# noway/nzcp-circom

Measured on AMD Instinct MI355X. Metric: groth16_proofs_per_sec_nzcp_live, higher is better.
Workload: dtype u32x8 (256-bit Montgomery integers); 1 GPU; nzcp_liveTest.circom = NZCPPubIdentity(1, 355, 0, 4, 2, 4, 6), single proof: nVars=825434, nConstraints=830227, nPublic=513, domain=2^20, nCoefs=4236306; parallelism=1gpu

## Files before the change

nzcp-circom_amd/csrc/internal.h:

```cpp
#pragma once
#include <hip/hip_runtime.h>
#include <stddef.h>
#include <stdint.h>
#include <stdlib.h>
#include <string.h>
#include <functional>
#include <memory>
#include <new>
#include <string>
#include <vector>

#include "../../include/g16_prover.h"
#include "device_job.h"
#include "ec.cuh"
#include "fq29.cuh"

struct g16_prover;
namespace g16 {

void set_error(const std::string& msg);
const char* get_error();

#define G16_HIP(expr)                                                                      \
  do {                                                                                     \
// ... 196 lines not shown
  uint64_t max_entries = 0;
};
size_t msm_point_bytes(int curve);
int msm_group_create(MsmGroup& g, const MsmSectionIn* secs, int nsec, const MsmConfig& cfg);
struct MsmWorkspaceDelete { void operator()(MsmWorkspace* ws) const; };
using MsmWorkspacePtr = std::unique_ptr<MsmWorkspace, MsmWorkspaceDelete>;
int msm_workspace_create(MsmWorkspacePtr& ws, const MsmGroup& g);
static constexpr int kMsmPrioHighest = -1000;
void msm_set_aux_stream_priority(int prio);
struct MsmResult {
  G1XYZZ g1[kMsmMaxSections];
  G2XYZZ g2;
};
static constexpr uint32_t kDupMin = 8;
static constexpr uint32_t kDupChunkBits = 16;
int msm_launch(const MsmGroup& g, MsmWorkspace* ws, const Fr* d_scalars, hipStream_t st, hipStream_t st2);
int msm_launch_front(const MsmGroup& g, MsmWorkspace* ws, const Fr* d_scalars, hipStream_t st);
int msm_launch_lanes(const MsmGroup& g, MsmWorkspace* ws, hipStream_t st, hipStream_t st2, hipEvent_t gate1,
                     hipEvent_t gate2);
void msm_set_quota(MsmWorkspace* ws, uint32_t quota_g1, uint32_t quota_g2);
hipEvent_t msm_event(MsmWorkspace* ws, int which);
int msm_collect(const MsmGroup& g, MsmWorkspace* ws, MsmResult* out,
                const std::function<void(const MsmResult&)>* after_g1 = nullptr);
double trace_ms();
float msm_last_accum_ms(const MsmWorkspace* ws, int lane);
void msm_set_throughput(MsmWorkspace* ws, const MsmGroup& g, bool on);
void msm_set_waves(MsmWorkspace* ws, uint32_t waves_g1, uint32_t waves_g2);
float msm_event_offset_ms(MsmWorkspace* ws, hipEvent_t base, int lane, int which);

template <class F> inline void msm_combine_windows(XYZZ<F>& total, const XYZZ<F>* windows, int W, int c, bool ones) {
  xyzz_set_inf(total);
  for (int j = W - 1; j >= 0; j--) {
    if (!xyzz_is_inf(total))
      for (int k = 0; k < c; k++) xyzz_dbl(total);
    xyzz_add(total, windows[j]);
  }
  if (ones) xyzz_add(total, windows[W]);
}
template <class F> inline void msm_add_bit_sums(XYZZ<F>& total, const XYZZ<F>* bits, uint32_t chunk_bits, uint32_t nrows) {
  XYZZ<F> acc;
  xyzz_set_inf(acc);
  for (int b = (int)nrows - 1; b >= 0; b--) {
    if (!xyzz_is_inf(acc))
      for (uint32_t k = 0; k < chunk_bits; k++) xyzz_dbl(acc);
    xyzz_add(acc, bits[b]);
  }
  xyzz_add(total, acc);
}
// ... 3 lines not shown
```

nzcp-circom_amd/csrc/msm.cuh:

```cuda
#pragma once
#include <stdlib.h>

#include <atomic>

#include "ec29.cuh"
#include "internal.h"

namespace g16 {

struct MsmPlan {
  uint32_t nsec, n;
  uint32_t sec_begin[kMsmMaxSections];
  int c, Ws;
  uint32_t W, pf, B, low_bits, bins, rps, rows, ones;
  uint32_t salt_bits;
  uint32_t dup_rows, dup_bits;
  uint32_t wb, wx;
  uint32_t wkb;
};
__host__ __device__ __forceinline__ uint32_t msm_win_off(const MsmPlan& pl, uint32_t j) { return j * pl.wb + (j < pl.wx ? j : pl.wx); }
__host__ __device__ __forceinline__ uint32_t msm_win_bits(const MsmPlan& pl, uint32_t j) { return pl.wb + (j < pl.wx ? 1u : 0u); }

__host__ __device__ __forceinline__ uint32_t msm_dup_hash(const uint32_t x[8], uint32_t bits) {
  uint64_t h = 0x9E3779B97F4A7C15ull;
// ... 29 lines not shown
  DeviceBuf<uint4> d_qdesc;
  DeviceBuf<uint32_t> d_class;
  DeviceBuf<uint32_t> d_queue;
  DeviceBuf<uint32_t> d_redo;
  DeviceBuf<void> d_partial;
  DeviceBuf<void> d_bsum;
  DeviceBuf<uint32_t> d_heavy;
  DeviceBuf<uint32_t> d_medium;
  uint32_t max_heavy = 0;
  DeviceBuf<void> d_seg;
  DeviceBuf<void> d_red;
  bool reduce_scan = false;
  void* d_canon = nullptr;
  DeviceBuf<void> d_canon_own;
  DeviceBuf<void> d_dseg;
  DeviceBuf<void> d_dred;
  DeviceEvent ev_dup_fork, ev_dup_join;
  DeviceBuf<uint32_t> d_dcount;
  DeviceBuf<uint32_t> d_dlist;
  uint32_t nsec_lane = 0;
  PinnedBuf<uint8_t> h_pinned;
  bool rows_mapped = false;
  size_t out_bytes = 0;
  DeviceEvent ev0, ev1;
  DeviceEvent ev_done;
  DeviceEvent trace_ev[4];
  DeviceStream st_dup;
  float last_accum_ms = 0.f;
  hipEvent_t gate = nullptr;
  uint32_t waves_per_simd = 0;
  uint32_t chunk_quota = 0;
};

struct MsmWorkspace {
  DeviceBuf<uint32_t> d_hist;
  DeviceBuf<uint32_t> d_bin_cnt;
  DeviceBuf<uint32_t> d_bin_start;
  DeviceBuf<uint2> d_tmp;
  DeviceBuf<uint32_t> d_sorted;
  DeviceBuf<uint32_t> d_cnt;
  uint32_t nb = 0;
  DeviceBuf<uint32_t> d_dup_cnt;
  DeviceBuf<uint32_t> d_dup_rep;
  DeviceBuf<uint32_t> d_dup_mixed;
  const Fr* d_scalars = nullptr;
  bool direct = false;
  uint32_t bin_cap = 0;
  uint32_t dup_chunk = 16, dup_bit_rows = 16;
  PinnedBuf<uint32_t> h_over;
  hipStream_t st_last = nullptr, st2_last = nullptr;
  MsmLaneWs lane[2];
// ... 728 lines not shown
  static_assert(sizeof(TPT) == sizeof(PT), "tail ops must share the point layout");
  static const bool trace = getenv("G16_TRACE_HOST") != nullptr;
  auto mark = [&](int k) {
    if (!trace) return;
    if (!ln.trace_ev[k]) (void)ln.trace_ev[k].create();
    (void)hipEventRecord(ln.trace_ev[k], st);
  };
  int rc = msm_build_queue(g, ws, ln, st);
  if (rc) return rc;
  mark(0);
  const uint32_t nbk = ln.key_hi - ln.key_lo;
  const uint32_t full_occ = (uint32_t)F::kAccumWavesPerSimd;
  const uint32_t occ = (ln.waves_per_simd && ln.waves_per_simd < full_occ) ? ln.waves_per_simd : full_occ;
  uint64_t waves = (uint64_t)256 * 4 * occ;
  const uint64_t max_chunks = (ln.max_tasks + kTaskChunk - 1) / kTaskChunk;
  uint32_t quota = 0xffffffffu;
  if (ln.chunk_quota) {
    quota = ln.chunk_quota;
    waves = (max_chunks + quota - 1) / quota + 64;
  }
  if (waves > max_chunks) waves = max_chunks;
  if (waves == 0) waves = 1;
  if (ln.gate) G16_HIP(hipStreamWaitEvent(st, ln.gate, 0));
  G16_HIP(hipEventRecord(ln.ev0, st));
  msm_accumulate_kernel<F><<<(unsigned)waves, 64, 0, st>>>((const PackedAffine<F>*)d_bases, ws->d_sorted, ln.d_toff, nbk,
                                                            ln.point_base, ln.d_qdesc, ln.d_queue, ln.d_redo,
                                                            (PT*)ln.d_partial, quota);
  G16_HIP(hipEventRecord(ln.ev1, st));
  msm_redo_kernel<F><<<64, 64, 0, st>>>((const PackedAffine<F>*)d_bases, ws->d_sorted, ln.point_base, ln.d_task_desc,
                                        ln.d_queue, ln.d_redo, (PT*)ln.d_partial);
  msm_combine_light_kernel<FT><<<(nbk + kTailThreads - 1) / kTailThreads, kTailThreads, 0, st>>>((const TPT*)ln.d_partial, ln.d_toff, nbk,
                                                              (TPT*)ln.d_bsum, ln.d_heavy, ln.max_heavy, ln.d_medium,
                                                              msm_light_max(ln), ln.h_stat);
  msm_combine_medium_kernel<FT><<<1024, kTailThreads, 0, st>>>((const TPT*)ln.d_partial, ln.d_toff, (TPT*)ln.d_bsum, ln.d_medium,
                                                              ln.max_heavy);
  msm_combine_heavy_kernel<FT><<<2048, kTailThreads, 0, st>>>((const TPT*)ln.d_partial, ln.d_toff, (TPT*)ln.d_bsum,
                                                   ln.d_heavy, ln.max_heavy);
  mark(1);
  uint32_t nout_pts = ln.row_pts;
  if (g.dup_rows) {
    hipStream_t sd = ln.st_dup ? ln.st_dup : st;
    if (sd != st) {
      G16_HIP(hipEventRecord(ln.ev_dup_fork, st));
      G16_HIP(hipStreamWaitEvent(sd, ln.ev_dup_fork, 0));
    }
    const uint32_t nchunk = (1u << g.dup_bits) >> 6, drows = ln.nsec_lane * ws->dup_bit_rows;
    const uint32_t waves_d = drows * nchunk;
    const uint32_t sec0 = ln.key_lo / (g.rps * g.B), dup_row0 = (uint32_t)g.W + (g.ones ? 1u : 0u);
    G16_HIP(hipMemsetAsync(ln.d_dcount, 0, 16, sd));
    msm_dup_compact_kernel<<<((ln.nsec_lane << g.dup_bits) + 255) / 256, 256, 0, sd>>>(
        ln.d_toff, g.B, g.rps, dup_row0, g.dup_bits, sec0, ln.nsec_lane, ws->d_dup_cnt, ws->d_dup_mixed, ln.d_dcount, ln.d_dlist);
// ... 68 lines not shown
```

nzcp-circom_amd/csrc/msm_g1.hip:

```cpp
#include <string.h>

#include "msm.cuh"

namespace g16 {

size_t msm_point_bytes(int curve) { return curve == 2 ? sizeof(G2XYZZ) : sizeof(G1XYZZ); }

__device__ __forceinline__ uint32_t msm_extract(const uint32_t s[8], int pos, int c) {
  const int word = pos >> 5, off = pos & 31;
  if (word >= 8) return 0;
  uint64_t v = s[word];
  if (word + 1 < 8) v |= (uint64_t)s[word + 1] << 32;
  return (uint32_t)(v >> off) & ((1u << c) - 1);
}

__device__ __forceinline__ bool msm_load_scalar(const Fr* __restrict__ scalars, const uint32_t* __restrict__ src,
                                                uint32_t g, const U256& K, uint32_t s[8], uint32_t* bits = nullptr) {
  const Fr x = scalars[src ? src[g] : g];
  uint32_t hi = 0;
#pragma unroll
  for (int k = 1; k < 8; k++) hi |= x.v[k];
  const bool one = (hi == 0 && x.v[0] == 1);
  if (bits) {
    uint32_t b = 0;
// ... 833 lines not shown
    out_pts += drows;
    G16_ALLOC(ln.d_dseg, drows * nchunk * pb + 256);
    G16_ALLOC(ln.d_dred, 2 * drows * ((nchunk + 63) / 64) * pb + 256);
    G16_ALLOC(ln.d_dcount, 64);
    if (curve == 2) {
      int plo = 0, phi = 0;
      G16_HIP(hipDeviceGetStreamPriorityRange(&plo, &phi));
      if (t_aux_prio != kMsmPrioHighest) phi = t_aux_prio;
      G16_STREAM(ln.st_dup, hipStreamNonBlocking, phi);
    }
    G16_EVENT_FLAGS(ln.ev_dup_fork, hipEventDisableTiming);
    G16_EVENT_FLAGS(ln.ev_dup_join, hipEventDisableTiming);
    G16_ALLOC(ln.d_dlist, ((size_t)ln.nsec_lane << g.dup_bits) * 4 + 64);
  }
  ln.out_bytes = out_pts * cpb;
  G16_PINNED(ln.h_pinned, ln.out_bytes + 256);
  ln.rows_mapped = !(getenv("G16_ROWS_COPY") && atoi(getenv("G16_ROWS_COPY")));
  if (ln.rows_mapped) {
    G16_HIP(hipHostGetDevicePointer(&ln.d_canon, ln.h_pinned, 0));
  } else {
    G16_HIP_AS(ln.d_canon_own.alloc_bytes(ln.out_bytes + 256), "hipMalloc(&ln.d_canon, ln.out_bytes + 256)");
    ln.d_canon = ln.d_canon_own;
  }
  G16_EVENT(ln.ev0);
  G16_EVENT(ln.ev1);
  G16_EVENT(ln.ev_done);
  return G16_OK;
}

void MsmWorkspaceDelete::operator()(MsmWorkspace* ws) const { delete ws; }

static int workspace_fill(MsmWorkspace* ws, const MsmGroup& g) {
  if (g.n == 0) return G16_OK;
  msm_set_throughput(ws, g, false);
  const uint32_t nrb = g.rows * g.bins;
  ws->nb = g.rows * g.B;
  G16_ALLOC(ws->d_hist, ((size_t)g.chunks * nrb + 4) * 4);
  G16_ALLOC(ws->d_bin_cnt, ((size_t)nrb + 4) * 4);
  G16_ALLOC(ws->d_bin_start, ((size_t)nrb + 4) * 4);
  {
    const bool off = getenv("G16_NO_DIRECT_BIN") && atoi(getenv("G16_NO_DIRECT_BIN"));
    uint64_t cap = (g.max_entries * 5 / 2) / nrb + 1024;
    if (const char* e = getenv("G16_TEST_BIN_CAP"))
      if (atoll(e) > 0) cap = (uint64_t)atoll(e);
    ws->direct = g.dense && g.nsec == 1 && !g.ones && !g.dup_rows && !off && cap * nrb < 0x7fffffffull;
    ws->bin_cap = ws->direct ? (uint32_t)cap : 0u;
  }
  G16_PINNED(ws->h_over, 64);
// ... 88 lines not shown
  const uint32_t ntiles = (nbk + kScanTile - 1) / kScanTile;
  if (!g.task_len_forced && ln.h_stat[0] > ln.h_stat[1]) {
    const uint64_t e = ln.h_stat[0] - ln.h_stat[1];
    ln.task_len = msm_task_len_for(e / (ln.curve == 2 ? 131072u : 262144u), ln.task_len_min);
  }
  msm_scan_tiles_kernel<<<ntiles, 256, 0, st>>>(cnt, nbk, ln.task_len, ln.d_tile_a, ln.d_tile_b, ln.d_tile_c);
  msm_scan_top_kernel<<<1, 1024, 0, st>>>(ln.d_tile_a, ln.d_tile_b, ln.d_tile_c, ntiles, off_base, ln.d_off + nbk,
                                          ln.d_toff + nbk, ln.d_foff + nbk, (uint32_t)ln.max_tasks,
                                          MsmSmallInit{ln.h_stat, ln.d_class, ln.d_queue, ln.d_heavy, ln.d_medium});
  msm_scan_apply_kernel<<<ntiles, 256, 0, st>>>(cnt, nbk, ln.task_len, ln.d_tile_a, ln.d_tile_b, ln.d_tile_c, off_base,
                                                ln.d_queue, ln.d_off, ln.d_toff, ln.d_foff, ln.d_class);
  msm_task_fill_kernel<<<(nbk + 255) / 256, 256, 0, st>>>(ln.d_off, ln.d_toff, ln.d_foff, nbk, ln.task_len, ln.d_task_desc,
                                                          ln.d_qdesc, ln.d_class, ln.d_class + kRemClasses,
                                                          (uint32_t)ln.max_tasks);
  G16_HIP(hipGetLastError());
  return G16_OK;
}

int msm_launch_front(const MsmGroup& g, MsmWorkspace* ws, const Fr* d_scalars, hipStream_t st) {
  ws->launched = true;
  ws->st_last = st;
  ws->st2_last = nullptr;
  ws->empty = (g.n == 0);
  for (auto& ln : ws->lane) ln.last_accum_ms = 0.f;
  if (g.n == 0) return G16_OK;
  return msm_front_end(g, ws, d_scalars, st);
}

int msm_launch_lanes(const MsmGroup& g, MsmWorkspace* ws, hipStream_t st, hipStream_t st2, hipEvent_t gate1,
                     hipEvent_t gate2) {
  if (g.n == 0) return G16_OK;
  int rc;
  ws->st2_last = st2;
  if (ws->lane[1].active) {
    hipStream_t s2 = st2 ? st2 : st;
    if (s2 != st) G16_HIP(hipStreamWaitEvent(s2, ws->ev_sorted, 0));
    ws->lane[1].gate = gate2;
    if ((rc = msm_launch_lane_g2(g, ws, ws->lane[1], s2))) return rc;
  }
  if (ws->lane[0].active) {
    ws->lane[0].gate = gate1;
    rc = msm_launch_lane_t<Fq29Ops>(g, ws, ws->lane[0], g.d_bases, st);
    if (rc) return rc;
  }
  return G16_OK;
}

int msm_launch(const MsmGroup& g, MsmWorkspace* ws, const Fr* d_scalars, hipStream_t st, hipStream_t st2) {
  int rc = msm_launch_front(g, ws, d_scalars, st);
  if (rc) return rc;
  return msm_launch_lanes(g, ws, st, st2, nullptr, nullptr);
}

hipEvent_t msm_event(MsmWorkspace* ws, int which) {
  switch (which) {
    case 0: return ws->ev_sorted;
    case 1: return ws->lane[0].ev0;
    case 2: return ws->lane[0].ev1;
    case 3: return ws->lane[0].active ? ws->lane[0].ev_done : nullptr;
    default: return ws->lane[1].active ? ws->lane[1].ev_done : nullptr;
  }
}

int msm_collect(const MsmGroup& g, MsmWorkspace* ws, MsmResult* out, const std::function<void(const MsmResult&)>* after_g1) {
  for (auto& p : out->g1) xyzz_set_inf(p);
  xyzz_set_inf(out->g2);
  if (!ws->launched || ws->empty) return G16_OK;
  bool overflow = false;
  for (int l = 0; l < 2; l++) {
    MsmLaneWs& ln = ws->lane[l];
    if (!ln.active) continue;
    G16_HIP(hipEventSynchronize(ln.ev_done));
    static const bool trace = getenv("G16_TRACE_HOST") != nullptr;
    if (trace) fprintf(stderr, "[g16 tail] %s lane %d: host saw its row sums at %.3f ms\n", g.dup_rows ? "W" : "H", l, trace_ms());
    (void)hipEventElapsedTime(&ln.last_accum_ms, ln.ev0, ln.ev1);
    if (ln.h_stat[2] || ln.h_stat[3]) {
      set_error(ln.h_stat[2] ? "msm: lane " + std::to_string(l) + " needed " + std::to_string(ln.h_stat[2]) +
                                   " bucket tasks, its buffers hold " + std::to_string(ln.max_tasks)
                             : "msm: lane " + std::to_string(l) + " overflowed its heavy-bucket list");
      overflow = true;
      continue;
    }
    if (g.dup_rows && getenv("G16_DEBUG_DUP")) {
      uint32_t dc[4] = {0, 0, 0, 0};
      (void)hipMemcpy(dc, ln.d_dcount, 16, hipMemcpyDeviceToHost);
      fprintf(stderr, "[g16 dup] lane %d: repeated-value buckets per section: %u %u %u\n", l, dc[0], dc[1], dc[2]);
    }
    const MsmReducePlan rp = msm_reduce_plan(g, ln);
    const uint32_t ngroups = (rp.nwg + kPairGroup - 1) / kPairGroup;
    if (l == 0) {
      const G1XYZZ* rows = reinterpret_cast<const G1XYZZ*>(ln.h_pinned.p);
      std::vector<G1XYZZ> folded;
      if (ln.reduce_scan && rp.nwg > kPairGroup) {
        folded.resize(ln.rows);
        for (uint32_t r = 0; r < ln.rows; r++)
          msm_fold_row<FqOps>(folded[r], rows + (size_t)r * ngroups * 3, ngroups, rp, msm_row_kind(rp, r));
      }
      const G1XYZZ* rsum = !folded.empty() ? folded.data() : rows;
      const bool merged = g.dup_rows && ws->dup_chunk == (uint32_t)g.c && ws->dup_bit_rows == (uint32_t)g.W;
      std::vector<G1XYZZ> wrow;
      for (int s = 0; s < g.nsec; s++) {
        const G1XYZZ* rs = rsum + (size_t)s * g.rps;
        const G1XYZZ* dup = rows + ln.row_pts + (size_t)s * ws->dup_bit_rows;
        if (merged) {
          wrow.assign(rs, rs + g.W + (g.ones ? 1 : 0));
          for (int j = 0; j < g.W; j++) xyzz_add(wrow[j], dup[j]);
          rs = wrow.data();
        }
        msm_combine_windows<FqOps>(out->g1[s], rs, g.W, g.c, g.ones);
        if (g.dup_rows && !merged) msm_add_bit_sums<FqOps>(out->g1[s], dup, ws->dup_chunk, ws->dup_bit_rows);
      }
      if (after_g1 && *after_g1) (*after_g1)(*out);
    } else {
      const G2XYZZ* rows = reinterpret_cast<const G2XYZZ*>(ln.h_pinned.p);
      std::vector<G2XYZZ> folded;
      if (ln.reduce_scan && rp.nwg > kPairGroup) {
        folded.resize(ln.rows);
        for (uint32_t r = 0; r < ln.rows; r++)
          msm_fold_row<Fq2Ops>(folded[r], rows + (size_t)r * ngroups * 3, ngroups, rp, msm_row_kind(rp, r));
      }
      const G2XYZZ* rsum = !folded.empty() ? folded.data() : rows;
      const bool merged = g.dup_rows && ws->dup_chunk == (uint32_t)g.c && ws->dup_bit_rows == (uint32_t)g.W;
      std::vector<G2XYZZ> wrow;
      if (merged) {
        wrow.assign(rsum, rsum + g.W + (g.ones ? 1 : 0));
        for (int j = 0; j < g.W; j++) xyzz_add(wrow[j], rows[ln.row_pts + j]);
        rsum = wrow.data();
      }
      msm_combine_windows<Fq2Ops>(out->g2, rsum, g.W, g.c, g.ones);
      if (g.dup_rows && !merged) msm_add_bit_sums<Fq2Ops>(out->g2, rows + ln.row_pts, ws->dup_chunk, ws->dup_bit_rows);
    }
  }
  if (overflow) return G16_E_STATE;
  if (ws->direct && ws->h_over[0]) {
    ws->direct = false;
    ws->h_over[0] = 0;
    int rc = msm_launch_front(g, ws, ws->d_scalars, ws->st_last);
    if (!rc) rc = msm_launch_lanes(g, ws, ws->st_last, ws->st2_last, nullptr, nullptr);
    if (rc) return rc;
    return msm_collect(g, ws, out, after_g1);
  }
  return G16_OK;
}

float msm_last_accum_ms(const MsmWorkspace* ws, int lane) { return ws->lane[lane & 1].last_accum_ms; }
void msm_set_throughput(MsmWorkspace* ws, const MsmGroup& g, bool on) {
  if (!ws) return;
  ws->dup_chunk = on ? g.dup_chunk_wide : g.dup_chunk;
  ws->dup_bit_rows = (254 + ws->dup_chunk - 1) / ws->dup_chunk;
  for (auto& ln : ws->lane)
    if (ln.active) ln.seg_len = on ? ln.seg_len_thr : ln.seg_len_lat;
}
void msm_set_waves(MsmWorkspace* ws, uint32_t waves_g1, uint32_t waves_g2) {
  ws->lane[0].waves_per_simd = waves_g1;
  ws->lane[1].waves_per_simd = waves_g2;
}
void msm_set_quota(MsmWorkspace* ws, uint32_t quota_g1, uint32_t quota_g2) {
  ws->lane[0].chunk_quota = quota_g1;
  ws->lane[1].chunk_quota = quota_g2;
}
float msm_event_offset_ms(MsmWorkspace* ws, hipEvent_t base, int lane, int which) {
  float t = 0.f;
  const MsmLaneWs& ln = ws->lane[lane & 1];
  hipEvent_t e = which < 4 ? ws->trace_ev[which] : which == 4 ? ln.ev0 : which == 5 ? ln.ev1 : ln.trace_ev[(which - 6) & 3];
  if (e && hipEventQuery(e) == hipSuccess) (void)hipEventElapsedTime(&t, base, e);
  return t;
}

}
```

nzcp-circom_amd/csrc/prover.cpp:

```cpp
#include <fcntl.h>
#include <stdio.h>
#include <stdlib.h>
#include <string.h>
#include <unistd.h>

#include <memory>
#include <mutex>

#include "../../include/g16_prover.h"
#include "binfile.h"
#include "internal.h"
#include "witness_program.h"

namespace g16 {

static thread_local std::string g_err;
void set_error(const std::string& msg) { g_err = msg; }
const char* get_error() { return g_err.c_str(); }

static int need_section(const BinView& f, uint32_t id, const char* name, BinSection& out) {
  out = f.sec[id];
  if (out.p) return G16_OK;
  set_error(std::string(name) + ": Missing section " + std::to_string(id));
  return G16_E_FORMAT;
}

static void g1_out(uint8_t out[64], const G1Affine& p) {
  Fq x = fp_from_mont(p.x), y = fp_from_mont(p.y);
  memcpy(out, x.v, 32);
  memcpy(out + 32, y.v, 32);
}
static void g2_out(uint8_t out[128], const G2Affine& p) {
  Fq v[4] = {fp_from_mont(p.x.a), fp_from_mont(p.x.b), fp_from_mont(p.y.a), fp_from_mont(p.y.b)};
// ... 45 lines not shown
    MsmWorkspacePtr ws[3];
    DeviceEvent evs[2][8];
    DeviceEvent mevs[2][3][2];
    g16_timings tms[2] = {};
    int set = 0;
    DeviceEvent* ev = evs[0];
    DeviceEvent (*mev)[2] = mevs[0];
    DeviceBuf<F29> d_a, d_b, d_c;
    DeviceBuf<F29> d_wm;
    DeviceBuf<Fr> d_p;
    DeviceBuf<Fr> d_w;
    DeviceBuf<uint32_t> d_flag;
    PinnedBuf<uint32_t> h_flag;
    DeviceStream st;
    DeviceStream wst2_own, wst_own;
  };
  static constexpr int kCtx = 3;
  int nctx = 3;
  g16_timings tm{};
  int tm_ctx = -1;
  int tm_set = 0;
  std::mutex mu;
  ProofCtx ctx[kCtx];

  ~g16_prover() { (void)hipSetDevice(device); }
};

static int check_device(int device) {
  int n = 0;
  if (hipGetDeviceCount(&n) != hipSuccess || n <= 0) {
    set_error("no HIP device available: libg16hip has no CPU fallback");
    return G16_E_NOGPU;
  }
  if (device < 0 || device >= n) { set_error("device ordinal out of range"); return G16_E_ARG; }
  G16_HIP(hipSetDevice(device));
  return G16_OK;
}

static void shard_range(uint32_t total, int rank, int count, uint32_t& lo, uint32_t& hi) {
  lo = (uint32_t)((uint64_t)total * rank / count);
  hi = (uint32_t)((uint64_t)total * (rank + 1) / count);
}

static int build_csr(g16_prover* P, const BinSection& s4) {
  if (s4.size < 4) { set_error("zkey: Invalid File format"); return G16_E_FORMAT; }
  const uint32_t nc = rd32(s4.p);
  if ((uint64_t)nc * 44 + 4 > s4.size) { set_error("zkey: Invalid File format"); return G16_E_FORMAT; }
  P->nCoefs = nc;
// ... 498 lines not shown
  uint32_t lo, hi;
  shard_range(P->N, P->shard_rank, P->shard_count, lo, hi);
  if ((rc = launch_join_h_front(P, c, lo, hi, fuse))) return rc;
  trace_host("h front end", th0);
  if ((rc = launch_witness_lanes(P, c, false))) return rc;
  trace_host("witness lanes", th0);
  if ((rc = launch_h_lanes(P, c, true))) return rc;
  trace_host("h lanes", th0);
  return G16_OK;
}

static int refresh_timings(g16_prover* P) {
  if (P->tm_ctx < 0) return G16_OK;
  ProofCtx& c = P->ctx[P->tm_ctx];
  const int set = P->tm_set;
  P->tm_ctx = -1;
  G16_HIP(hipSetDevice(P->device));
  const DeviceEvent* ev = c.evs[set];
  const DeviceEvent (*mev)[2] = c.mevs[set];
  G16_HIP(hipEventSynchronize(ev[5]));
  G16_HIP(hipEventSynchronize(mev[0][1]));
  if (P->b2_solo) G16_HIP(hipEventSynchronize(mev[2][1]));
  g16_timings t = c.tms[set];
  float wg = 0.f, hg = 0.f;
  const hipEvent_t span[5][2] = {{ev[2], ev[3]}, {ev[3], ev[4]}, {ev[2], ev[5]}, {mev[0][0], mev[0][1]}, {mev[1][0], mev[1][1]}};
  float* dst[5] = {&t.qap_ms, &t.ntt_ms, &t.total_ms, &wg, &hg};
  for (int k = 0; k < 5; k++) {
    const hipError_t e = hipEventElapsedTime(dst[k], span[k][0], span[k][1]);
    if (e != hipSuccess) {
      set_error(std::string("g16_get_timings: hipEventElapsedTime: ") + hipGetErrorString(e));
      return G16_E_HIP;
    }
  }
  const float g2 = msm_event_offset_ms(c.ws[P->b2_solo ? 2 : 0].get(), mev[P->b2_solo ? 2 : 0][0], 1, 9);
  t.msm_ms[0] = wg; t.msm_ms[1] = 0.f; t.msm_ms[2] = g2; t.msm_ms[3] = 0.f; t.msm_ms[4] = hg;
  static const bool trace_dev = getenv("G16_TRACE_HOST") != nullptr;
  if (trace_dev) {
    float t_ntt0 = 0, t_ntt1 = 0;
    (void)hipEventElapsedTime(&t_ntt0, ev[2], ev[3]);
    (void)hipEventElapsedTime(&t_ntt1, ev[2], ev[4]);
    fprintf(stderr, "[g16 dev] qap 0..%.3f  ntt+join ..%.3f  total %.3f\n", t_ntt0, t_ntt1, t.total_ms);
    static const char* nm[2] = {"W", "H"};
    for (int gi = 0; gi < 2; gi++) {
      float s0 = 0, s1 = 0;
      (void)hipEventElapsedTime(&s0, ev[2], mev[gi][0]);
      (void)hipEventElapsedTime(&s1, ev[2], mev[gi][1]);
      auto off = [&](int lane, int k) { return msm_event_offset_ms(c.ws[gi].get(), ev[2], lane, k); };
      fprintf(stderr, "[g16 dev] %s  start %.3f pass0 %.3f binscan %.3f pass1 %.3f binsort+scans %.3f | G1 queue %.3f accumulate "
              "%.3f..%.3f combine %.3f reduce %.3f end %.3f (stream end %.3f)\n", nm[gi], s0, off(0, 0), off(0, 1), off(0, 2),
              off(0, 3), off(0, 6), off(0, 4), off(0, 5), off(0, 7), off(0, 8), off(0, 9), s1);
      if (gi == 0)
        fprintf(stderr, "[g16 dev] W2 (G2 lane) queue %.3f accumulate %.3f..%.3f combine %.3f reduce %.3f end %.3f\n",
                off(1, 6), off(1, 4), off(1, 5), off(1, 7), off(1, 8), off(1, 9));
    }
  }
  t.upload_ms = P->tm.upload_ms;
  P->tm = t;
  return G16_OK;
}

static void next_event_set(g16_prover* P, ProofCtx& c) {
  const int ci = (int)(&c - P->ctx), ns = c.set ^ 1;
  if (P->tm_ctx == ci && P->tm_set == ns) (void)refresh_timings(P);
  c.set = ns;
  c.ev = c.evs[ns];
  c.mev = c.mevs[ns];
  c.tms[ns] = g16_timings{};
}
static void mark_completed(g16_prover* P, ProofCtx& c) {
  P->tm_ctx = (int)(&c - P->ctx);
  P->tm_set = c.set;
  static const bool trace_dev = getenv("G16_TRACE_HOST") != nullptr;
  if (trace_dev) (void)refresh_timings(P);
}

static int collect_witness_msms(g16_prover* P, ProofCtx& c, Partial& out,
                                const std::function<void(const MsmResult&)>* after_g1 = nullptr) {
  MsmResult r;
  int rc = msm_collect(P->grp[0], c.ws[0].get(), &r, after_g1);
  if (rc) return rc;
  out.A = r.g1[0];
  out.B1 = r.g1[1];
  out.C = r.g1[2];
  out.B2 = r.g2;
  g16_timings& tm = c.tms[c.set];
  tm.msm_accum_kernel_ms[0] = msm_last_accum_ms(c.ws[0].get(), 0);
  tm.msm_accum_kernel_ms[1] = tm.msm_accum_kernel_ms[3] = 0.f;
  tm.msm_accum_kernel_ms[2] = msm_last_accum_ms(c.ws[0].get(), 1);
  if (P->b2_solo) {
    if ((rc = msm_collect(P->grp[2], c.ws[2].get(), &r))) return rc;
    out.B2 = r.g2;
    tm.msm_accum_kernel_ms[2] = msm_last_accum_ms(c.ws[2].get(), 1);
  }
  return G16_OK;
}
static int collect_h_msm(g16_prover* P, ProofCtx& c, Partial& out) {
  MsmResult r;
  int rc = msm_collect(P->grp[1], c.ws[1].get(), &r);
  if (rc) return rc;
  out.H = r.g1[0];
  trace_tail("H sum folded");
  c.tms[c.set].msm_accum_kernel_ms[4] = msm_last_accum_ms(c.ws[1].get(), 0);
  return G16_OK;
}
static int collect_ctx(g16_prover* P, ProofCtx& c, Partial& out) {
  const int rc = collect_witness_msms(P, c, out);
  const int rch = collect_h_msm(P, c, out);
  return rc ? rc : rch;
}
static void drain_ctx(g16_prover* P, ProofCtx& c) {
  const std::string err = get_error();
  (void)hipSetDevice(P->device);
  Partial part;
  (void)collect_ctx(P, c, part);
  (void)hipStreamSynchronize(c.st);
  if (c.wst != c.st) (void)hipStreamSynchronize(c.wst);
  if (c.wst2 != c.st) (void)hipStreamSynchronize(c.wst2);
  set_error(err);
}
static int collect_and_assemble(g16_prover* P, ProofCtx& c, const Blinding& bl, g16_proof* out) {
  Partial part;
  EarlyTail e;
  bool g1_half = false;
  const std::function<void(const MsmResult&)> after_g1 = [&](const MsmResult& r) {
    assemble_early_g1(&P->kp, bl, r.g1[0], r.g1[1], e);
    g1_half = true;
    trace_tail("G1 sums folded, pi_a and the pi_c terms assembled");
  };
  int rc = collect_witness_msms(P, c, part, &after_g1);
  trace_tail("witness sums folded");
  if (!rc) {
    if (!g1_half) assemble_early_g1(&P->kp, bl, part.A, part.B1, e);
    assemble_early_g2(&P->kp, bl, part.B2, e);
  }
  trace_tail("pi_a, pi_b assembled");
  const int rch = collect_h_msm(P, c, part);
  trace_tail("H sum folded, streams drained");
  if (rc) return rc;
  if (rch) return rch;
  assemble_late(e, part.C, part.H, out);
  trace_tail("pi_c assembled");
  return G16_OK;
}

static int device_impl(g16_prover* P, uint32_t slot, Partial& out) {
  if (slot >= P->slot_dev.size() || !P->slot_dev[slot]) { set_error("witness slot not staged"); return G16_E_STATE; }
  int rc = launch_ctx(P, P->ctx[0], P->slot_dev[slot]);
  if (rc) { drain_ctx(P, P->ctx[0]); return rc; }
  if ((rc = collect_ctx(P, P->ctx[0], out))) return rc;
  mark_completed(P, P->ctx[0]);
  return G16_OK;
}

static int shard_guard(const g16_prover* P) {
  if (!P->shard_begun) return G16_OK;
  set_error("g16_shard_begin in progress: call g16_shard_end first");
// ... 140 lines not shown
    for (size_t k = 0; k < nctx; k++) {
      if (!busy[k]) continue;
      ProofCtx& c = p->ctx[k];
      hipEvent_t evs[4] = {c.ev[3], c.ws[0] ? msm_event(c.ws[0].get(), 3) : nullptr, c.ws[0] ? msm_event(c.ws[0].get(), 4) : nullptr,
                           p->b2_solo && c.ws[2] ? msm_event(c.ws[2].get(), 4) : nullptr};
      for (hipEvent_t e : evs)
        if (e)
          if (int rc = wcalc_chunk_release(d, e)) return rc;
    }
    return G16_OK;
  }
};

extern "C" {

const char* g16_last_error(void) { return get_error(); }

int g16_create(const uint8_t* zkey, size_t zkey_len, const g16_opts* opts, g16_prover** out) {
  if (!out) { set_error("out is NULL"); return G16_E_ARG; }
  *out = nullptr;
  std::unique_ptr<g16_prover> P(new g16_prover());
  int rc = create_impl(zkey, zkey_len, opts, P.get());
  if (rc) return rc;
  *out = P.release();
  return G16_OK;
}

void g16_destroy(g16_prover* p) { delete p; }

int g16_stage_witness(g16_prover* p, uint32_t slot, const uint8_t* wtns, size_t wtns_len) {
  if (!p) { set_error("prover is NULL"); return G16_E_ARG; }
  std::lock_guard<std::mutex> lk(p->mu);
  if (int rc = shard_guard(p)) return rc;
  return stage_impl(p, slot, wtns, wtns_len);
}

int g16_prove_partial(g16_prover* p, uint32_t slot, uint8_t partial[G16_PARTIAL_BYTES]) {
  if (!p || !partial) { set_error("NULL argument"); return G16_E_ARG; }
  std::lock_guard<std::mutex> lk(p->mu);
  if (int rc = shard_guard(p)) return rc;
  Partial part;
  int rc = device_impl(p, slot, part);
  if (rc) return rc;
  memcpy(partial, &part, sizeof(part));
  return G16_OK;
}
// ... 68 lines not shown
  if (slot >= p->slot_pub.size()) { set_error("witness slot not staged"); return G16_E_STATE; }
  if (count != (uint32_t)p->shard_count) {
    set_error("g16_prove_finish: expected " + std::to_string(p->shard_count) + " partial sums, got " + std::to_string(count));
    return G16_E_ARG;
  }
  std::vector<Partial> parts(count);
  memcpy(parts.data(), partials, (size_t)count * sizeof(Partial));
  int rc = finish_impl(&p->kp, parts.data(), count, r, s, out);
  if (!rc && pub && p->nPublic) memcpy(pub, p->slot_pub[slot].data(), (size_t)p->nPublic * 32);
  return rc;
}

static int prove_staged_locked(g16_prover* p, uint32_t slot, const uint8_t r[32], const uint8_t s[32], g16_proof* out,
                               uint8_t* pub, bool mark = true) {
  if (p->shard_count != 1) { set_error("sharded handle: use g16_prove_partial/g16_prove_finish"); return G16_E_STATE; }
  if (slot >= p->slot_dev.size() || !p->slot_dev[slot]) { set_error("witness slot not staged"); return G16_E_STATE; }
  Blinding bl;
  int rc = launch_ctx(p, p->ctx[0], p->slot_dev[slot]);
  const int rcb = prepare_blinding(&p->kp, r, s, bl);
  if (rc || rcb) {
    drain_ctx(p, p->ctx[0]);
    return rc ? rc : rcb;
  }
  rc = collect_and_assemble(p, p->ctx[0], bl, out);
  if (rc) return rc;
  if (mark) mark_completed(p, p->ctx[0]);
  if (pub && p->nPublic) memcpy(pub, p->slot_pub[slot].data(), (size_t)p->nPublic * 32);
  return G16_OK;
}

int g16_prove_staged(g16_prover* p, uint32_t slot, const uint8_t r[32], const uint8_t s[32], g16_proof* out,
                     uint8_t* pub) {
  if (!p || !out) { set_error("NULL argument"); return G16_E_ARG; }
  std::lock_guard<std::mutex> lk(p->mu);
  if (int rc = shard_guard(p)) return rc;
  return prove_staged_locked(p, slot, r, s, out, pub);
}

int g16_stage_inputs(g16_prover* p, uint32_t slot, g16_wtns_calculator* h, const uint8_t* inputs, size_t n_inputs, uint32_t* status) {
  if (!p || !h || !status || (n_inputs && !inputs)) { set_error("NULL argument"); return G16_E_ARG; }
  std::lock_guard<std::mutex> lk(p->mu);
  if (int rc = shard_guard(p)) return rc;
  if (int rc = wcalc_match_prover(h, "stage inputs", p->device, p->nVars, p->nPublic)) return rc;
  if (slot >= 65536) { set_error("slot out of range"); return G16_E_ARG; }
  if (int rc = wcalc_check_inputs(h, inputs, n_inputs, 1)) return rc;
  G16_HIP(hipSetDevice(p->device));
  if (p->slot_dev.size() <= slot) { p->slot_dev.resize(slot + 1); p->slot_pub.resize(slot + 1); }
// ... 224 lines not shown
```

Baseline: 281.3 proofs/s.

## Fold G2 witness MSM sums on a helper thread beside G1 fold

Adds a persistent helper thread with a handoff queue. While the main thread waits on and folds the G1 lane's row sums, the helper collects and folds the G2 lane and assembles pi_b, so the two host-side tail folds overlap. The MSM collect is split into per-lane and finish steps, and the accumulate-kernel timing events are double-buffered per context set and read when timings are gathered. The cost is thread synchronisation overhead, more complex error handling, and concurrent HIP calls from two host threads.

```diff
diff --git a/nzcp-circom_amd/csrc/fold_handoff.h b/nzcp-circom_amd/csrc/fold_handoff.h
--- /dev/null
+++ b/nzcp-circom_amd/csrc/fold_handoff.h
@@ -0,0 +1,70 @@
+#pragma once
+#include <condition_variable>
+#include <functional>
+#include <mutex>
+#include <string>
+#include <utility>
+
+namespace g16 {
+
+class FoldHandoff {
+ public:
+  using Job = std::function<int(std::string& err)>;
+
+  void post(Job job) {
+    {
+      std::lock_guard<std::mutex> lk(mu_);
+      job_ = std::move(job);
+      err_.clear();
+      state_ = kPosted;
+    }
+    cv_.notify_all();
+  }
+  int wait(std::string* err = nullptr) {
+    std::unique_lock<std::mutex> lk(mu_);
+    cv_.wait(lk, [&] { return state_ == kDone; });
+    state_ = kIdle;
+    if (err) *err = err_;
+    return rc_;
+  }
+  bool serve_one() {
+    Job job;
+    {
+      std::unique_lock<std::mutex> lk(mu_);
+      cv_.wait(lk, [&] { return state_ == kPosted || stop_; });
+      if (state_ != kPosted) return false;
+      job = std::move(job_);
+      job_ = nullptr;
+      state_ = kRunning;
+    }
+    std::string err;
+    const int rc = job(err);
+    {
+      std::lock_guard<std::mutex> lk(mu_);
+      rc_ = rc;
+      err_ = std::move(err);
+      state_ = kDone;
+    }
+    cv_.notify_all();
+    return true;
+  }
+  void stop() {
+    {
+      std::lock_guard<std::mutex> lk(mu_);
+      stop_ = true;
+    }
+    cv_.notify_all();
+  }
+
+ private:
+  enum State { kIdle, kPosted, kRunning, kDone };
+  std::mutex mu_;
+  std::condition_variable cv_;
+  State state_ = kIdle;
+  bool stop_ = false;
+  Job job_;
+  int rc_ = 0;
+  std::string err_;
+};
+
+}
diff --git a/nzcp-circom_amd/csrc/internal.h b/nzcp-circom_amd/csrc/internal.h
--- a/nzcp-circom_amd/csrc/internal.h
+++ b/nzcp-circom_amd/csrc/internal.h
@@ -242,8 +242,12 @@
 hipEvent_t msm_event(MsmWorkspace* ws, int which);
 int msm_collect(const MsmGroup& g, MsmWorkspace* ws, MsmResult* out,
                 const std::function<void(const MsmResult&)>* after_g1 = nullptr);
+int msm_collect_lane(const MsmGroup& g, MsmWorkspace* ws, int lane, MsmResult* out);
+int msm_collect_finish(const MsmGroup& g, MsmWorkspace* ws, MsmResult* out, bool* redone,
+                       const std::function<void(const MsmResult&)>* after_g1 = nullptr);
 double trace_ms();
-float msm_last_accum_ms(const MsmWorkspace* ws, int lane);
+void msm_set_event_set(MsmWorkspace* ws, int set);
+int msm_accum_ms(const MsmWorkspace* ws, int lane, int set, float* ms);
 void msm_set_throughput(MsmWorkspace* ws, const MsmGroup& g, bool on);
 void msm_set_waves(MsmWorkspace* ws, uint32_t waves_g1, uint32_t waves_g2);
 float msm_event_offset_ms(MsmWorkspace* ws, hipEvent_t base, int lane, int which);
diff --git a/nzcp-circom_amd/csrc/msm.cuh b/nzcp-circom_amd/csrc/msm.cuh
--- a/nzcp-circom_amd/csrc/msm.cuh
+++ b/nzcp-circom_amd/csrc/msm.cuh
@@ -75,11 +75,11 @@
   PinnedBuf<uint8_t> h_pinned;
   bool rows_mapped = false;
   size_t out_bytes = 0;
-  DeviceEvent ev0, ev1;
+  DeviceEvent ev0[2], ev1[2];
+  int es = 0;
   DeviceEvent ev_done;
   DeviceEvent trace_ev[4];
   DeviceStream st_dup;
-  float last_accum_ms = 0.f;
   hipEvent_t gate = nullptr;
   uint32_t waves_per_simd = 0;
   uint32_t chunk_quota = 0;
@@ -854,11 +854,11 @@
   if (waves > max_chunks) waves = max_chunks;
   if (waves == 0) waves = 1;
   if (ln.gate) G16_HIP(hipStreamWaitEvent(st, ln.gate, 0));
-  G16_HIP(hipEventRecord(ln.ev0, st));
+  G16_HIP(hipEventRecord(ln.ev0[ln.es], st));
   msm_accumulate_kernel<F><<<(unsigned)waves, 64, 0, st>>>((const PackedAffine<F>*)d_bases, ws->d_sorted, ln.d_toff, nbk,
                                                             ln.point_base, ln.d_qdesc, ln.d_queue, ln.d_redo,
                                                             (PT*)ln.d_partial, quota);
-  G16_HIP(hipEventRecord(ln.ev1, st));
+  G16_HIP(hipEventRecord(ln.ev1[ln.es], st));
   msm_redo_kernel<F><<<64, 64, 0, st>>>((const PackedAffine<F>*)d_bases, ws->d_sorted, ln.point_base, ln.d_task_desc,
                                         ln.d_queue, ln.d_redo, (PT*)ln.d_partial);
   msm_combine_light_kernel<FT><<<(nbk + kTailThreads - 1) / kTailThreads, kTailThreads, 0, st>>>((const TPT*)ln.d_partial, ln.d_toff, nbk,
diff --git a/nzcp-circom_amd/csrc/msm_g1.hip b/nzcp-circom_amd/csrc/msm_g1.hip
--- a/nzcp-circom_amd/csrc/msm_g1.hip
+++ b/nzcp-circom_amd/csrc/msm_g1.hip
@@ -879,8 +879,10 @@
     G16_HIP_AS(ln.d_canon_own.alloc_bytes(ln.out_bytes + 256), "hipMalloc(&ln.d_canon, ln.out_bytes + 256)");
     ln.d_canon = ln.d_canon_own;
   }
-  G16_EVENT(ln.ev0);
-  G16_EVENT(ln.ev1);
+  for (int k = 0; k < 2; k++) {
+    G16_EVENT(ln.ev0[k]);
+    G16_EVENT(ln.ev1[k]);
+  }
   G16_EVENT(ln.ev_done);
   return G16_OK;
 }
@@ -1015,7 +1017,6 @@
   ws->st_last = st;
   ws->st2_last = nullptr;
   ws->empty = (g.n == 0);
-  for (auto& ln : ws->lane) ln.last_accum_ms = 0.f;
   if (g.n == 0) return G16_OK;
   return msm_front_end(g, ws, d_scalars, st);
 }
@@ -1048,95 +1049,113 @@
 hipEvent_t msm_event(MsmWorkspace* ws, int which) {
   switch (which) {
     case 0: return ws->ev_sorted;
-    case 1: return ws->lane[0].ev0;
-    case 2: return ws->lane[0].ev1;
+    case 1: return ws->lane[0].ev0[ws->lane[0].es];
+    case 2: return ws->lane[0].ev1[ws->lane[0].es];
     case 3: return ws->lane[0].active ? ws->lane[0].ev_done : nullptr;
     default: return ws->lane[1].active ? ws->lane[1].ev_done : nullptr;
   }
 }
 
+int msm_collect_lane(const MsmGroup& g, MsmWorkspace* ws, int l, MsmResult* out) {
+  if (l == 0) for (auto& p : out->g1) xyzz_set_inf(p);
+  else xyzz_set_inf(out->g2);
+  if (!ws->launched || ws->empty) return G16_OK;
+  MsmLaneWs& ln = ws->lane[l];
+  if (!ln.active) return G16_OK;
+  G16_HIP(hipEventSynchronize(ln.ev_done));
+  static const bool trace = getenv("G16_TRACE_HOST") != nullptr;
+  if (trace) fprintf(stderr, "[g16 tail] %s lane %d: host saw its row sums at %.3f ms\n", g.dup_rows ? "W" : "H", l, trace_ms());
+  if (ln.h_stat[2] || ln.h_stat[3]) {
+    set_error(ln.h_stat[2] ? "msm: lane " + std::to_string(l) + " needed " + std::to_string(ln.h_stat[2]) +
+                                 " bucket tasks, its buffers hold " + std::to_string(ln.max_tasks)
+                           : "msm: lane " + std::to_string(l) + " overflowed its heavy-bucket list");
+    return G16_E_STATE;
+  }
+  if (g.dup_rows && getenv("G16_DEBUG_DUP")) {
+    uint32_t dc[4] = {0, 0, 0, 0};
+    (void)hipMemcpy(dc, ln.d_dcount, 16, hipMemcpyDeviceToHost);
+    fprintf(stderr, "[g16 dup] lane %d: repeated-value buckets per section: %u %u %u\n", l, dc[0], dc[1], dc[2]);
+  }
+  const MsmReducePlan rp = msm_reduce_plan(g, ln);
+  const uint32_t ngroups = (rp.nwg + kPairGroup - 1) / kPairGroup;
+  if (l == 0) {
+    const G1XYZZ* rows = reinterpret_cast<const G1XYZZ*>(ln.h_pinned.p);
+    std::vector<G1XYZZ> folded;
+    if (ln.reduce_scan && rp.nwg > kPairGroup) {
+      folded.resize(ln.rows);
+      for (uint32_t r = 0; r < ln.rows; r++)
+        msm_fold_row<FqOps>(folded[r], rows + (size_t)r * ngroups * 3, ngroups, rp, msm_row_kind(rp, r));
+    }
+    const G1XYZZ* rsum = !folded.empty() ? folded.data() : rows;
+    const bool merged = g.dup_rows && ws->dup_chunk == (uint32_t)g.c && ws->dup_bit_rows == (uint32_t)g.W;
+    std::vector<G1XYZZ> wrow;
+    for (int s = 0; s < g.nsec; s++) {
+      const G1XYZZ* rs = rsum + (size_t)s * g.rps;
+      const G1XYZZ* dup = rows + ln.row_pts + (size_t)s * ws->dup_bit_rows;
+      if (merged) {
+        wrow.assign(rs, rs + g.W + (g.ones ? 1 : 0));
+        for (int j = 0; j < g.W; j++) xyzz_add(wrow[j], dup[j]);
+        rs = wrow.data();
+      }
+      msm_combine_windows<FqOps>(out->g1[s], rs, g.W, g.c, g.ones);
+      if (g.dup_rows && !merged) msm_add_bit_sums<FqOps>(out->g1[s], dup, ws->dup_chunk, ws->dup_bit_rows);
+    }
+  } else {
+    const G2XYZZ* rows = reinterpret_cast<const G2XYZZ*>(ln.h_pinned.p);
+    std::vector<G2XYZZ> folded;
+    if (ln.reduce_scan && rp.nwg > kPairGroup) {
+      folded.resize(ln.rows);
+      for (uint32_t r = 0; r < ln.rows; r++)
+        msm_fold_row<Fq2Ops>(folded[r], rows + (size_t)r * ngroups * 3, ngroups, rp, msm_row_kind(rp, r));
+    }
+    const G2XYZZ* rsum = !folded.empty() ? folded.data() : rows;
+    const bool merged = g.dup_rows && ws->dup_chunk == (uint32_t)g.c && ws->dup_bit_rows == (uint32_t)g.W;
+    std::vector<G2XYZZ> wrow;
+    if (merged) {
+      wrow.assign(rsum, rsum + g.W + (g.ones ? 1 : 0));
+      for (int j = 0; j < g.W; j++) xyzz_add(wrow[j], rows[ln.row_pts + j]);
+      rsum = wrow.data();
+    }
+    msm_combine_windows<Fq2Ops>(out->g2, rsum, g.W, g.c, g.ones);
+    if (g.dup_rows && !merged) msm_add_bit_sums<Fq2Ops>(out->g2, rows + ln.row_pts, ws->dup_chunk, ws->dup_bit_rows);
+  }
+  return G16_OK;
+}
+
+int msm_collect_finish(const MsmGroup& g, MsmWorkspace* ws, MsmResult* out, bool* redone,
+                       const std::function<void(const MsmResult&)>* after_g1) {
+  if (redone) *redone = false;
+  if (!ws->launched || ws->empty || !ws->direct || !ws->h_over[0]) return G16_OK;
+  ws->direct = false;
+  ws->h_over[0] = 0;
+  if (redone) *redone = true;
+  int rc = msm_launch_front(g, ws, ws->d_scalars, ws->st_last);
+  if (!rc) rc = msm_launch_lanes(g, ws, ws->st_last, ws->st2_last, nullptr, nullptr);
+  if (rc) return rc;
+  return msm_collect(g, ws, out, after_g1);
+}
+
 int msm_collect(const MsmGroup& g, MsmWorkspace* ws, MsmResult* out, const std::function<void(const MsmResult&)>* after_g1) {
-  for (auto& p : out->g1) xyzz_set_inf(p);
-  xyzz_set_inf(out->g2);
-  if (!ws->launched || ws->empty) return G16_OK;
-  bool overflow = false;
-  for (int l = 0; l < 2; l++) {
-    MsmLaneWs& ln = ws->lane[l];
-    if (!ln.active) continue;
-    G16_HIP(hipEventSynchronize(ln.ev_done));
-    static const bool trace = getenv("G16_TRACE_HOST") != nullptr;
-    if (trace) fprintf(stderr, "[g16 tail] %s lane %d: host saw its row sums at %.3f ms\n", g.dup_rows ? "W" : "H", l, trace_ms());
-    (void)hipEventElapsedTime(&ln.last_accum_ms, ln.ev0, ln.ev1);
-    if (ln.h_stat[2] || ln.h_stat[3]) {
-      set_error(ln.h_stat[2] ? "msm: lane " + std::to_string(l) + " needed " + std::to_string(ln.h_stat[2]) +
-                                   " bucket tasks, its buffers hold " + std::to_string(ln.max_tasks)
-                             : "msm: lane " + std::to_string(l) + " overflowed its heavy-bucket list");
-      overflow = true;
-      continue;
-    }
-    if (g.dup_rows && getenv("G16_DEBUG_DUP")) {
-      uint32_t dc[4] = {0, 0, 0, 0};
-      (void)hipMemcpy(dc, ln.d_dcount, 16, hipMemcpyDeviceToHost);
-      fprintf(stderr, "[g16 dup] lane %d: repeated-value buckets per section: %u %u %u\n", l, dc[0], dc[1], dc[2]);
-    }
-    const MsmReducePlan rp = msm_reduce_plan(g, ln);
-    const uint32_t ngroups = (rp.nwg + kPairGroup - 1) / kPairGroup;
-    if (l == 0) {
-      const G1XYZZ* rows = reinterpret_cast<const G1XYZZ*>(ln.h_pinned.p);
-      std::vector<G1XYZZ> folded;
-      if (ln.reduce_scan && rp.nwg > kPairGroup) {
-        folded.resize(ln.rows);
-        for (uint32_t r = 0; r < ln.rows; r++)
-          msm_fold_row<FqOps>(folded[r], rows + (size_t)r * ngroups * 3, ngroups, rp, msm_row_kind(rp, r));
-      }
-      const G1XYZZ* rsum = !folded.empty() ? folded.data() : rows;
-      const bool merged = g.dup_rows && ws->dup_chunk == (uint32_t)g.c && ws->dup_bit_rows == (uint32_t)g.W;
-      std::vector<G1XYZZ> wrow;
-      for (int s = 0; s < g.nsec; s++) {
-        const G1XYZZ* rs = rsum + (size_t)s * g.rps;
-        const G1XYZZ* dup = rows + ln.row_pts + (size_t)s * ws->dup_bit_rows;
-        if (merged) {
-          wrow.assign(rs, rs + g.W + (g.ones ? 1 : 0));
-          for (int j = 0; j < g.W; j++) xyzz_add(wrow[j], dup[j]);
-          rs = wrow.data();
-        }
-        msm_combine_windows<FqOps>(out->g1[s], rs, g.W, g.c, g.ones);
-        if (g.dup_rows && !merged) msm_add_bit_sums<FqOps>(out->g1[s], dup, ws->dup_chunk, ws->dup_bit_rows);
-      }
-      if (after_g1 && *after_g1) (*after_g1)(*out);
-    } else {
-      const G2XYZZ* rows = reinterpret_cast<const G2XYZZ*>(ln.h_pinned.p);
-      std::vector<G2XYZZ> folded;
-      if (ln.reduce_scan && rp.nwg > kPairGroup) {
-        folded.resize(ln.rows);
-        for (uint32_t r = 0; r < ln.rows; r++)
-          msm_fold_row<Fq2Ops>(folded[r], rows + (size_t)r * ngroups * 3, ngroups, rp, msm_row_kind(rp, r));
-      }
-      const G2XYZZ* rsum = !folded.empty() ? folded.data() : rows;
-      const bool merged = g.dup_rows && ws->dup_chunk == (uint32_t)g.c && ws->dup_bit_rows == (uint32_t)g.W;
-      std::vector<G2XYZZ> wrow;
-      if (merged) {
-        wrow.assign(rsum, rsum + g.W + (g.ones ? 1 : 0));
-        for (int j = 0; j < g.W; j++) xyzz_add(wrow[j], rows[ln.row_pts + j]);
-        rsum = wrow.data();
-      }
-      msm_combine_windows<Fq2Ops>(out->g2, rsum, g.W, g.c, g.ones);
-      if (g.dup_rows && !merged) msm_add_bit_sums<Fq2Ops>(out->g2, rows + ln.row_pts, ws->dup_chunk, ws->dup_bit_rows);
-    }
-  }
-  if (overflow) return G16_E_STATE;
-  if (ws->direct && ws->h_over[0]) {
-    ws->direct = false;
-    ws->h_over[0] = 0;
-    int rc = msm_launch_front(g, ws, ws->d_scalars, ws->st_last);
-    if (!rc) rc = msm_launch_lanes(g, ws, ws->st_last, ws->st2_last, nullptr, nullptr);
-    if (rc) return rc;
-    return msm_collect(g, ws, out, after_g1);
-  }
+  const int rc0 = msm_collect_lane(g, ws, 0, out);
+  if (rc0 && rc0 != G16_E_STATE) return rc0;
+  if (!rc0 && after_g1 && *after_g1 && ws->launched && !ws->empty && ws->lane[0].active) (*after_g1)(*out);
+  const int rc1 = msm_collect_lane(g, ws, 1, out);
+  if (rc1) return rc1;
+  if (rc0) return rc0;
+  return msm_collect_finish(g, ws, out, nullptr, after_g1);
+}
+
+int msm_accum_ms(const MsmWorkspace* ws, int lane, int set, float* ms) {
+  *ms = 0.f;
+  const MsmLaneWs& ln = ws->lane[lane & 1];
+  if (ws->empty || !ws->launched || !ln.active) return G16_OK;
+  G16_HIP(hipEventElapsedTime(ms, ln.ev0[set & 1], ln.ev1[set & 1]));
   return G16_OK;
 }
-
-float msm_last_accum_ms(const MsmWorkspace* ws, int lane) { return ws->lane[lane & 1].last_accum_ms; }
+void msm_set_event_set(MsmWorkspace* ws, int set) {
+  if (!ws) return;
+  for (auto& ln : ws->lane) ln.es = set & 1;
+}
 void msm_set_throughput(MsmWorkspace* ws, const MsmGroup& g, bool on) {
   if (!ws) return;
   ws->dup_chunk = on ? g.dup_chunk_wide : g.dup_chunk;
@@ -1155,7 +1174,7 @@
 float msm_event_offset_ms(MsmWorkspace* ws, hipEvent_t base, int lane, int which) {
   float t = 0.f;
   const MsmLaneWs& ln = ws->lane[lane & 1];
-  hipEvent_t e = which < 4 ? ws->trace_ev[which] : which == 4 ? ln.ev0 : which == 5 ? ln.ev1 : ln.trace_ev[(which - 6) & 3];
+  hipEvent_t e = which < 4 ? ws->trace_ev[which] : which == 4 ? ln.ev0[ln.es] : which == 5 ? ln.ev1[ln.es] : ln.trace_ev[(which - 6) & 3];
   if (e && hipEventQuery(e) == hipSuccess) (void)hipEventElapsedTime(&t, base, e);
   return t;
 }
diff --git a/nzcp-circom_amd/csrc/prover.cpp b/nzcp-circom_amd/csrc/prover.cpp
--- a/nzcp-circom_amd/csrc/prover.cpp
+++ b/nzcp-circom_amd/csrc/prover.cpp
@@ -6,9 +6,11 @@
 
 #include <memory>
 #include <mutex>
+#include <thread>
 
 #include "../../include/g16_prover.h"
 #include "binfile.h"
+#include "fold_handoff.h"
 #include "internal.h"
 #include "witness_program.h"
 
@@ -100,8 +102,22 @@
   int tm_set = 0;
   std::mutex mu;
   ProofCtx ctx[kCtx];
-
-  ~g16_prover() { (void)hipSetDevice(device); }
+  FoldHandoff fold;
+  std::thread fold_thread;
+
+  void start_helper() {
+    fold_thread = std::thread([this] {
+      (void)hipSetDevice(device);
+      while (fold.serve_one()) {}
+    });
+  }
+  ~g16_prover() {
+    if (fold_thread.joinable()) {
+      fold.stop();
+      fold_thread.join();
+    }
+    (void)hipSetDevice(device);
+  }
 };
 
 static int check_device(int device) {
@@ -646,6 +662,13 @@
   G16_HIP(hipEventSynchronize(mev[0][1]));
   if (P->b2_solo) G16_HIP(hipEventSynchronize(mev[2][1]));
   g16_timings t = c.tms[set];
+  {
+    int rc;
+    if ((rc = msm_accum_ms(c.ws[0].get(), 0, set, &t.msm_accum_kernel_ms[0]))) return rc;
+    if ((rc = msm_accum_ms(c.ws[P->b2_solo ? 2 : 0].get(), 1, set, &t.msm_accum_kernel_ms[2]))) return rc;
+    if ((rc = msm_accum_ms(c.ws[1].get(), 0, set, &t.msm_accum_kernel_ms[4]))) return rc;
+    t.msm_accum_kernel_ms[1] = t.msm_accum_kernel_ms[3] = 0.f;
+  }
   float wg = 0.f, hg = 0.f;
   const hipEvent_t span[5][2] = {{ev[2], ev[3]}, {ev[3], ev[4]}, {ev[2], ev[5]}, {mev[0][0], mev[0][1]}, {mev[1][0], mev[1][1]}};
   float* dst[5] = {&t.qap_ms, &t.ntt_ms, &t.total_ms, &wg, &hg};
@@ -690,6 +713,7 @@
   c.ev = c.evs[ns];
   c.mev = c.mevs[ns];
   c.tms[ns] = g16_timings{};
+  for (auto& w : c.ws) msm_set_event_set(w.get(), ns);
 }
 static void mark_completed(g16_prover* P, ProofCtx& c) {
   P->tm_ctx = (int)(&c - P->ctx);
@@ -707,14 +731,9 @@
   out.B1 = r.g1[1];
   out.C = r.g1[2];
   out.B2 = r.g2;
-  g16_timings& tm = c.tms[c.set];
-  tm.msm_accum_kernel_ms[0] = msm_last_accum_ms(c.ws[0].get(), 0);
-  tm.msm_accum_kernel_ms[1] = tm.msm_accum_kernel_ms[3] = 0.f;
-  tm.msm_accum_kernel_ms[2] = msm_last_accum_ms(c.ws[0].get(), 1);
   if (P->b2_solo) {
     if ((rc = msm_collect(P->grp[2], c.ws[2].get(), &r))) return rc;
     out.B2 = r.g2;
-    tm.msm_accum_kernel_ms[2] = msm_last_accum_ms(c.ws[2].get(), 1);
   }
   return G16_OK;
 }
@@ -724,7 +743,6 @@
   if (rc) return rc;
   out.H = r.g1[0];
   trace_tail("H sum folded");
-  c.tms[c.set].msm_accum_kernel_ms[4] = msm_last_accum_ms(c.ws[1].get(), 0);
   return G16_OK;
 }
 static int collect_ctx(g16_prover* P, ProofCtx& c, Partial& out) {
@@ -742,20 +760,69 @@
   if (c.wst2 != c.st) (void)hipStreamSynchronize(c.wst2);
   set_error(err);
 }
-static int collect_and_assemble(g16_prover* P, ProofCtx& c, const Blinding& bl, g16_proof* out) {
+static int collect_witness_beside(g16_prover* P, ProofCtx& c, const Blinding& bl, Partial& part, EarlyTail& e) {
+  const MsmGroup& g = P->grp[0];
+  MsmWorkspace* ws = c.ws[0].get();
+  MsmResult r1, r2;
+  const auto origin = g_trace_origin;
+  struct Joined {
+    FoldHandoff& f;
+    bool waited = false;
+    int wait(std::string* err) { waited = true; return f.wait(err); }
+    ~Joined() { if (!waited) (void)f.wait(); }
+  } joined{P->fold};
+  P->fold.post([&, origin](std::string& err) -> int {
+    g_trace_origin = origin;
+    const int rc = no_bad_alloc("g16_prove: fold helper", [&]() -> int {
+      G16_HIP(hipSetDevice(P->device));
+      if (int rl = msm_collect_lane(g, ws, 1, &r2)) return rl;
+      assemble_early_g2(&P->kp, bl, r2.g2, e);
+      trace_tail("(helper) G2 sum folded, pi_b assembled");
+      return G16_OK;
+    });
+    if (rc) err = get_error();
+    return rc;
+  });
+  const int rc1 = msm_collect_lane(g, ws, 0, &r1);
+  if (!rc1) {
+    assemble_early_g1(&P->kp, bl, r1.g1[0], r1.g1[1], e);
+    trace_tail("G1 sums folded, pi_a and the pi_c terms assembled");
+  }
+  std::string err2;
+  const int rc2 = joined.wait(&err2);
+  if (rc2) set_error(err2);
+  if (rc1 || rc2) return (rc1 && rc1 != G16_E_STATE) ? rc1 : (rc2 ? rc2 : rc1);
+  r1.g2 = r2.g2;
+  bool redone = false;
+  if (int rc = msm_collect_finish(g, ws, &r1, &redone)) return rc;
+  part.A = r1.g1[0];
+  part.B1 = r1.g1[1];
+  part.C = r1.g1[2];
+  part.B2 = r1.g2;
+  if (redone) assemble_early(&P->kp, bl, part.A, part.B1, part.B2, e);
+  return G16_OK;
+}
+
+static int collect_and_assemble(g16_prover* P, ProofCtx& c, const Blinding& bl, g16_proof* out, bool beside = false) {
   Partial part;
   EarlyTail e;
-  bool g1_half = false;
-  const std::function<void(const MsmResult&)> after_g1 = [&](const MsmResult& r) {
-    assemble_early_g1(&P->kp, bl, r.g1[0], r.g1[1], e);
-    g1_half = true;
-    trace_tail("G1 sums folded, pi_a and the pi_c terms assembled");
-  };
-  int rc = collect_witness_msms(P, c, part, &after_g1);
-  trace_tail("witness sums folded");
-  if (!rc) {
-    if (!g1_half) assemble_early_g1(&P->kp, bl, part.A, part.B1, e);
-    assemble_early_g2(&P->kp, bl, part.B2, e);
+  int rc;
+  if (beside && !P->b2_solo && P->fold_thread.joinable()) {
+    rc = collect_witness_beside(P, c, bl, part, e);
+    trace_tail("witness sums folded");
+  } else {
+    bool g1_half = false;
+    const std::function<void(const MsmResult&)> after_g1 = [&](const MsmResult& r) {
+      assemble_early_g1(&P->kp, bl, r.g1[0], r.g1[1], e);
+      g1_half = true;
+      trace_tail("G1 sums folded, pi_a and the pi_c terms assembled");
+    };
+    rc = collect_witness_msms(P, c, part, &after_g1);
+    trace_tail("witness sums folded");
+    if (!rc) {
+      if (!g1_half) assemble_early_g1(&P->kp, bl, part.A, part.B1, e);
+      assemble_early_g2(&P->kp, bl, part.B2, e);
+    }
   }
   trace_tail("pi_a, pi_b assembled");
   const int rch = collect_h_msm(P, c, part);
@@ -942,6 +1009,7 @@
   std::unique_ptr<g16_prover> P(new g16_prover());
   int rc = create_impl(zkey, zkey_len, opts, P.get());
   if (rc) return rc;
+  P->start_helper();
   *out = P.release();
   return G16_OK;
 }
@@ -1056,7 +1124,7 @@
     drain_ctx(p, p->ctx[0]);
     return rc ? rc : rcb;
   }
-  rc = collect_and_assemble(p, p->ctx[0], bl, out);
+  rc = collect_and_assemble(p, p->ctx[0], bl, out, true);
   if (rc) return rc;
   if (mark) mark_completed(p, p->ctx[0]);
   if (pub && p->nPublic) memcpy(pub, p->slot_pub[slot].data(), (size_t)p->nPublic * 32);
```

After: 284.2 proofs/s, median of 6. +1.0%, better.
